# arjunchandra/paac

Measured on AMD Instinct MI355X. Metric: global env-steps/sec at 32 envs, t_max=5, Nature net; 1/2/4/8 MI355X, higher is better.
Workload: dtype f32; 1 GPU; breakout action set (A=4), NATURE net, 32 envs per GPU x 1 GPU, t_max=5, synthetic 84x84x4 u8 frames generated on device, sampler=numpy, hipGraph replay; envs_per_gpu=32, t_max=5, global_envs=32, parallelism=env-sharded dp1, no collective (one process)

## Files before the change

### __graft_entry__.py

```python
import os
import sys

ROOT = os.path.dirname(os.path.abspath(__file__))
if ROOT not in sys.path:
    sys.path.insert(0, ROOT)


USER_ARCHS = [
    "16,32,32,256",
    "32:8:4,64:5:2,64:3:1,512",
    "32:8:4,48:4:2,512",
    "16:8:4,16:4:1,256",
    "32:12:4,64:2:3,64:3:1,768",
    "16:4:2,32:1:1,48:5:5,1024",
    "32:8:4,64:4:2,64:8:1,512",
    "64:16:4,128:3:2,96:3:2,256",
]


def build():
    from concurrent.futures import ThreadPoolExecutor
    from paac_amd import build as b
    lib = b.build(verbose=False)
    with ThreadPoolExecutor(max_workers=4) as ex:
        list(ex.map(lambda spec: b.build_user_arch(*b.parse_user_arch(spec)), USER_ARCHS))
    from paac_amd import _lib
    _lib.load()
    assert os.path.exists(lib)
    import paac_amd.train


def smoke():
    import numpy as np
    import torch
    from oracle import network as onet
    from paac_amd import hip_ops
    assert torch.cuda.is_available(), "smoke() needs cuda:0"
    arch, A, B = "NATURE", 4, 40
    for weight_scale in (1.0, 3.5):
        rs = np.random.RandomState(0)
        params = {k: (v * weight_scale).astype(np.float32) for k, v in onet.init_params(arch, A, rs, dtype=np.float32).items()}
        states = rs.randint(0, 256, (B, 84, 84, 4)).astype(np.uint8)
        idx = rs.randint(0, A, B).astype(np.int32)
        y = rs.randn(B).astype(np.float32)
        adv = rs.randn(B).astype(np.float32)
        ctx = hip_ops.Context(1, A, max_batch=B)
        flat = np.zeros(ctx.layout["total"], dtype=np.float32)
        for t in ctx.layout["tensors"]:
            flat[t["offset"]:t["offset"] + t["size"]] = params[t["name"]].reshape(-1)
        p = torch.from_numpy(flat).cuda()
        s = torch.from_numpy(states).cuda()
        logits = torch.zeros((B, A), device="cuda")
        values = torch.zeros(B, device="cuda")
        grad = torch.zeros(ctx.layout["total"], device="cuda")
        ctx.forward(p, s, logits=logits, values=values)
        ctx.loss_backward(p, s, torch.from_numpy(idx).cuda(), torch.from_numpy(y).cuda(), torch.from_numpy(adv).cuda(), 0.02, grad)
        torch.cuda.synchronize()
        masks = {"a%d" % i: ctx.debug_activation(i, B).cpu().numpy() > 0 for i in (1, 2, 3)}
        masks["h"] = ctx.debug_activation(4, B).cpu().numpy() > 0
        L, g = onet.loss_and_grads(params, states, np.eye(A)[idx], y, adv, 0.02, arch, dtype=np.float64, relu_masks=masks)
        if weight_scale != 1.0:
            assert np.abs(L["logits"]).max() > 3.0 and np.abs(L["v"]).max() > 3.0
        assert np.abs(logits.cpu().numpy() - L["logits"]).max() < 1e-4
        assert np.abs(values.cpu().numpy() - L["v"]).max() < 1e-4
        gh = grad.cpu().numpy()
        gn = onet.global_norm(g)
        for t in ctx.layout["tensors"]:
            err = np.abs(gh[t["offset"]:t["offset"] + t["size"]] - g[t["name"]].reshape(-1)).max()
            assert err < 1e-4 * max(np.abs(g[t["name"]]).max(), 1e-3 * gn), (t["name"], err)
        ctx.close()
    print("smoke ok: logits/values within 1e-4, gradients within 1e-4 relative (initialisation-scale and trained-scale weights)")


if __name__ == "__main__":
    build()
    if len(sys.argv) > 1 and sys.argv[1] == "smoke":
        smoke()
```

### paac_amd/build.py

```python
import fcntl
import os
import subprocess
import sys
from concurrent.futures import ThreadPoolExecutor

HERE = os.path.dirname(os.path.abspath(__file__))
CSRC = os.path.join(HERE, "csrc")
LIB = os.path.join(HERE, "libpaac_hip.so")
SOURCES = ["api.hip", "net_fwd.hip", "net_bwd.hip", "misc.hip"]
HEADERS = sorted(f for f in os.listdir(CSRC) if f.endswith(".h")) + [os.path.join("..", "..", "include", "paac_hip.h")]
FLAGS = ["-O3", "-std=c++17", "--offload-arch=gfx950", "-fPIC", "-Wall", "-Wno-unused-function",
         "-Wno-unused-variable", "-Wno-unused-but-set-variable"]


def _stale(target, deps):
    if not os.path.exists(target):
        return True
    t = os.path.getmtime(target)
    return any(os.path.getmtime(d) > t for d in deps)


def build(force=False, verbose=True, extra_flags=(), lib_path=None, obj_suffix=""):
    lib = lib_path or LIB
    with open(lib + ".lock", "w") as lock:
        fcntl.flock(lock, fcntl.LOCK_EX)
        try:
            return _build_locked(force, verbose, extra_flags, lib, obj_suffix)
        finally:
            fcntl.flock(lock, fcntl.LOCK_UN)


def _build_locked(force, verbose, extra_flags, lib, obj_suffix):
    hipcc = os.environ.get("HIPCC", "/opt/rocm/bin/hipcc")
    hdrs = [os.path.join(CSRC, h) for h in HEADERS] + [os.path.abspath(__file__)]
    objs, jobs = [], []
    for src in SOURCES:
        s = os.path.join(CSRC, src)
        o = os.path.join(CSRC, src.replace(".hip", obj_suffix + ".o"))
        objs.append(o)
        if force or _stale(o, [s] + hdrs):
            jobs.append([hipcc] + FLAGS + list(extra_flags) + ["-c", s, "-o", o])

    def run(cmd):
        at = cmd.index("-o") + 1
        target = cmd[at]
        tmp = "%s.tmp.%d" % (target, os.getpid())
        cmd = cmd[:at] + [tmp] + cmd[at + 1:]
        try:
            _run(cmd)
            os.replace(tmp, target)
        finally:
            if os.path.exists(tmp):
                os.remove(tmp)

    def _run(cmd):
        if verbose:
            print(" ".join(cmd), flush=True)
        r = subprocess.run(cmd, capture_output=True, text=True)
        if r.returncode != 0:
            raise RuntimeError("hipcc failed:\n%s\n%s" % (" ".join(cmd), r.stderr[-8000:]))
        if verbose and r.stderr.strip():
            print(r.stderr[-4000:], file=sys.stderr)

    with ThreadPoolExecutor(max_workers=4) as ex:
        list(ex.map(run, jobs))
    if jobs or force or _stale(lib, objs):
        run([hipcc, "--offload-arch=gfx950", "-shared", "-fPIC", "-o", lib] + objs)
    return lib


def parse_user_arch(spec):
    parts = str(spec).split(",")
    convs = []
    for i, p in enumerate(parts[:-1]):
        v = [int(x) for x in p.split(":")]
        if len(v) == 1:
            if i >= len(FAMILY):
                raise ValueError("more than three layers in %r" % (spec,))
            v = [v[0]] + list(FAMILY[i])
        if len(v) != 3:
            raise ValueError("layer %r: expected filters or filters:size:stride" % (p,))
        convs.append(tuple(v))
    return convs, int(parts[-1])


FAMILY = [(8, 4), (4, 2), (3, 1)]


def user_arch_library(convs, fc):
    convs = [tuple(int(v) for v in c) for c in convs]
    tag = "_".join(str(f) for f, _, _ in convs) + "_%d" % fc
    if any((k, s) != FAMILY[i] for i, (_, k, s) in enumerate(convs)):
        tag += "_k" + "_".join("%dx%d" % (k, s) for _, k, s in convs)
    return os.path.join(HERE, "libpaac_hip_user_%s.so" % tag), "_user_" + tag


def build_user_arch(convs, fc, verbose=False):
    convs = [tuple(int(v) for v in c) for c in convs]
    if len(convs) not in (2, 3) or any(len(c) != 3 for c in convs):
        raise NotImplementedError("user architectures have two or three conv layers (filters, size, stride); got %r" % (convs,))
    if any(f % 16 or f < 16 for f, _, _ in convs) or fc % 256 or fc < 256:
        raise NotImplementedError("filter counts must be multiples of 16 and the fc width a multiple of 256 (MFMA tiles); "
                                  "got %r, fc %d" % (convs, fc))
    if any(k < 1 or s < 1 for _, k, s in convs):
        raise ValueError("kernel sizes and strides must be positive; got %r" % (convs,))
    if (convs[0][1] * 4) % 16:
        raise NotImplementedError("the first layer's kernel size must be 4, 8, 12 or 16 (kernel width x 4 input channels is "
                                  "read in MFMA K groups of 16); got %d" % convs[0][1])
    size = 84
    for _, k, s in convs:
        if size < k:
            raise ValueError("layer shapes %r leave no output (VALID convolutions over 84 x 84)" % (convs,))
        size = (size - k) // s + 1
    lib, suffix = user_arch_library(convs, fc)
    flags = ["-DPAAC_USER_ARCH", "-DPAAC_USER_NCONV=%d" % len(convs), "-DPAAC_USER_C1=%d" % convs[0][0],
             "-DPAAC_USER_C2=%d" % convs[1][0], "-DPAAC_USER_C3=%d" % (convs[2][0] if len(convs) == 3 else 0),
             "-DPAAC_USER_H=%d" % fc]
    layers = convs + [(0, 3, 1)] * (3 - len(convs))
    flags += ["-DPAAC_USER_K%d=%d" % (i + 1, k) for i, (_, k, _) in enumerate(layers)]
    flags += ["-DPAAC_USER_S%d=%d" % (i + 1, st) for i, (_, _, st) in enumerate(layers)]
    try:
        return build(verbose=verbose, extra_flags=flags, lib_path=lib, obj_suffix=suffix)
    except RuntimeError as exc:
        raise RuntimeError("building the user architecture %s (fc %d) failed: %s" % (convs, fc, exc)) from exc


if __name__ == "__main__":
    if "--user-arch" in sys.argv:
        spec = sys.argv[sys.argv.index("--user-arch") + 1]
        print(build_user_arch(*parse_user_arch(spec), verbose=True))
    elif "--stamps" in sys.argv or "--ksplit" in sys.argv:
        tag = ("_stamps" if "--stamps" in sys.argv else "") + ("_ksplit" if "--ksplit" in sys.argv else "")
        flags = (["-DPAAC_DMM_STAMPS"] if "--stamps" in sys.argv else []) + (["-DPAAC_T_ROLES=0"] if "--ksplit" in sys.argv else [])
        print(build(extra_flags=flags, lib_path=os.path.join(HERE, "libpaac_hip%s.so" % tag), obj_suffix=tag))
    else:
        print(build(force="--force" in sys.argv))
```

### paac_amd/csrc/net_fwd.hip

```cpp
#include "net_common.h"
#include "tower.h"
#include "tower2.h"
#include "fc_heads.h"
#include "gemm3.h"

namespace paac {

#ifdef PAAC_DMM_STAMPS
unsigned long long* g_tower_stamps = nullptr;
extern "C" void paac_debug_set_tower_stamps(unsigned long long* p) { g_tower_stamps = p; }
unsigned long long* g_stamps = nullptr;
int g_stamp_which = -1, g_stamp_calls = 0;
extern "C" void paac_debug_set_stamps(unsigned long long* p, int which) {
  g_stamps = p;
  g_stamp_which = which;
  g_stamp_calls = 0;
}
#endif

template <class G, bool U8, int NDIM, int EPI>
static int launch_fwd(const GemmArgs& g, Tune t, hipStream_t s) {
  constexpr int VN = (NDIM % 64 == 0) ? 4 : (NDIM % 32 == 0) ? 2 : 1;
  int cfg = t.cfg, ksplit = 1, xcd = t.xcd;
  if constexpr (EPI == EPI_SLAB) {
    ksplit = t.ksplit > 0 ? t.ksplit : 0;
    if (ksplit <= 0) {
      const long tiles = (long)((g.M + 15) / 16) * ((g.N + 16 * VN - 1) / (16 * VN));
      ksplit = pick_ksplit(tiles, 4, (g.K + 15) / 16, FC_SPLITS_MAX, 768);
    }
    if (ksplit > FC_SPLITS_MAX) ksplit = FC_SPLITS_MAX;
  }
  if (cfg < 0) {
    const long w = (long)((g.M + 15) / 16) * ((g.N + 16 * VN - 1) / (16 * VN)) * ksplit;
    cfg = (w <= 256) ? 0 : (w <= 1024) ? 3 : (w <= 4096) ? 4 : 5;
    if (U8) cfg += kExactBf16;
    xcd = -1;
  }
  if constexpr (U8) {
    if (cfg >= kExactBf16) {
      switch (cfg - kExactBf16) {
#define X(id, TM, NWM, WK, PF) \
  case id: launch_dmm<Dmm<G, U8, FRAG_K, FRAG_MN, TM, VN, NWM, 1, WK, 1, EPI, false, PF, 1>>(g, ksplit, ksplit, xcd, s); break;
        PAAC_FWD_CFGS(X)
#undef X
        default: break;
      }
      return ksplit;
    }
  }
  if constexpr (!U8 && VN == 4 && EPI == EPI_BIAS_RELU) {
    if (cfg >= kNarrow) {
      switch (cfg - kNarrow) {
#define X(id, TM, NWM, WK, PF) \
  case id: launch_dmm<Dmm<G, U8, FRAG_K, FRAG_MN, TM, 2, NWM, 1, WK, 1, EPI, false, PF>>(g, ksplit, ksplit, xcd, s); return ksplit;
        PAAC_FWD_NARROW_CFGS(X)
#undef X
        default: cfg -= kNarrow; break;
      }
    }
  }
  if (cfg >= kNarrow) cfg -= kNarrow;
  if constexpr (!U8) {
    if (cfg >= kSplitBf16) {
      switch (cfg - kSplitBf16) {
#define X(id, TM, NWM, WK, PF) \
  case id: launch_dmm<Dmm<G, U8, FRAG_K, FRAG_MN, TM, VN, NWM, 1, WK, 1, EPI, false, split_pf(PF), 2>>(g, ksplit, ksplit, xcd, s); return ksplit;
        PAAC_FWD_SPLIT_CFGS(X)
#undef X
        default: cfg -= kSplitBf16; break;
      }
    }
  }
  switch (cfg) {
#define X(id, TM, NWM, WK, PF) \
  case id: launch_dmm<Dmm<G, U8, FRAG_K, FRAG_MN, TM, VN, NWM, 1, WK, 1, EPI, false, PF>>(g, ksplit, ksplit, xcd, s); break;
    PAAC_FWD_CFGS(X)
#undef X
    default: break;
  }
  return ksplit;
}

static int launch_fc_gemm3(const float* x, const float* wf, float* slab, int batch, int K, int H, hipStream_t s) {
  static const int min_rows = env_int("PAAC_GEMM3_MIN_ROWS", 513);
  if (batch < min_rows || (K % 32) != 0) return 0;
  Gemm3Args a;
  memset(&a, 0, sizeof(a));
  a.A = x; a.lda = K;
  a.B = wf; a.ldb = H;
  a.out = slab; a.ldo = H;
  a.M = batch; a.N = H; a.K = K;
  using D = Gemm3<true, false, EPI_SLAB>;
  a.MB = (batch + D::TM - 1) / D::TM;
  a.NB = (H + D::TN - 1) / D::TN;
  const int stages = K / 32, tiles = a.MB * a.NB;
  int S = (256 + tiles / 2) / tiles;
  S = S < 1 ? 1 : (S > FC_SPLITS_MAX ? FC_SPLITS_MAX : S);
  a.stages_per_split = (stages + S - 1) / S;
  a.S = (stages + a.stages_per_split - 1) / a.stages_per_split;
  a.slab_stride = (long)batch * H;
  prof_mix(6);
  launch_k(gemm3_kernel<D>, dim3((unsigned)(a.MB * a.NB * a.S)), dim3(D::THREADS), s, PROF_WHOLE, a);
  return a.S;
}

size_t tower_pack_bytes() { return (size_t)kTowerPackAllVecs * sizeof(bf16x8); }
constexpr bool kTower2 = OtherNet::NCONV == 2 && OtherNet::C1 == 16 && OtherNet::C2 == 32 && OtherNet::FLAT == kT2Flat;
bool tower2_available() { return kTower2; }

int launch_pack_weights(paac_ctx* ctx, const float* params, hipStream_t s) {
  const paac_layout& L = ctx->layout;
  {
    const float* wf = params + L.offset[2 * ctx->spec.nconv];
    f32x4* out = reinterpret_cast<f32x4*>(ctx->fc_pack);
    if (ctx->cfg.arch == PAAC_ARCH_NATURE)
      launch_k(pack_fc_kernel<NatureNet::FLAT, NatureNet::H>, dim3((NatureNet::FLAT / 16) * (NatureNet::H / 16) * 64 / 256),
               dim3(256), s, PROF_NONE, wf, out);
    else
      launch_k(pack_fc_kernel<OtherNet::FLAT, OtherNet::H>, dim3((OtherNet::FLAT / 16) * (OtherNet::H / 16) * 64 / 256), dim3(256),
               s, PROF_NONE, wf, out);
  }
  if (ctx->tower2_on) {
    constexpr int threads2 = (8 * 1 + 8 * 2) * 64;
    launch_k(pack_tower2_kernel, dim3((threads2 + 255) / 256), dim3(256), s, PROF_NONE, params + L.offset[0], params + L.offset[2],
             reinterpret_cast<bf16x8*>(ctx->tower_pack));
    return 0;
  }
  if (!ctx->tower_on) return 0;
  constexpr int threads = (8 * 2 + 16 * 4 + 18 * 4) * 64;
  launch_k(pack_tower_kernel, dim3((threads + 255) / 256), dim3(256), s, PROF_NONE, params + L.offset[0], params + L.offset[2],
           params + L.offset[4], reinterpret_cast<bf16x8*>(ctx->tower_pack));
  return launch_pack_dgrad(ctx, params, s);
}

template <class G, bool KEEP>
static void launch_tower_variant(const TowerArgs& a, hipStream_t s) {
  launch_k(tower_kernel<G, KEEP>, dim3((unsigned)(a.batch * G::NR)), dim3(512), s, PROF_WHOLE, a);
}

static void launch_tower(paac_ctx* ctx, Workspace& W, const float* params, const uint8_t* states, int batch, bool keep,
                         bool packed3, hipStream_t s, Workspace* keepW = nullptr, int keep_row = 0) {
  const paac_layout& L = ctx->layout;
  TowerArgs a;
  a.states = states;
  const bf16x8* pk = reinterpret_cast<const bf16x8*>(ctx->tower_pack);
  a.w1p = pk;
  a.w2p = pk + kTowerW1Vecs;
  a.w3p = pk + kTowerW1Vecs + kTowerW2Vecs;
  a.b1 = params + L.offset[1];
  a.b2 = params + L.offset[3];
  a.b3 = params + L.offset[5];
  a.act1 = W.act[0];
  a.act2 = W.act[1];
  a.act3 = W.act[2];
  a.batch = batch;
  a.act3_packed = packed3 ? 1 : 0;
  a.act3_rows = nullptr;
  if (keepW) {
    keep = true;
    a.act1 = keepW->act[0] + (size_t)keep_row * 400 * NatureNet::C1;
    a.act2 = keepW->act[1] + (size_t)keep_row * 81 * NatureNet::C2;
    if (packed3) a.act3_rows = keepW->act[2] + (size_t)keep_row * NatureNet::FLAT;
    else a.act3 = keepW->act[2] + (size_t)keep_row * NatureNet::FLAT;
  }
#ifdef PAAC_DMM_STAMPS
  a.stamps = g_tower_stamps;
#endif
  const int force = ctx->tune[OP_CONV_TOWER][batch_class(batch)].cfg;
  int regions = (8 * batch <= 256) ? 8 : (4 * batch <= 256) ? 4 : (2 * batch <= 256) ? 2 : 1;
  if (force == 1 || force == 2 || force == 4 || force == 8) regions = force;
  if (regions == 8) {
    if (keep) launch_tower_variant<TowerGeom<4, 2>, true>(a, s);
    else launch_tower_variant<TowerGeom<4, 2>, false>(a, s);
  } else if (regions == 4) {
    if (keep) launch_tower_variant<TowerGeom<4, 4>, true>(a, s);
    else launch_tower_variant<TowerGeom<4, 4>, false>(a, s);
  } else if (regions == 2) {
    if (keep) launch_tower_variant<TowerGeom<4, 7>, true>(a, s);
    else launch_tower_variant<TowerGeom<4, 7>, false>(a, s);
  } else {
    if (keep) launch_tower_variant<TowerGeom<7, 7>, true>(a, s);
    else launch_tower_variant<TowerGeom<7, 7>, false>(a, s);
  }
}

template <class G, bool KEEP>
static void launch_tower2_variant(const Tower2Args& a, hipStream_t s) {
  launch_k(tower2_kernel<G, KEEP>, dim3((unsigned)(a.batch * G::NR)), dim3(512), s, PROF_WHOLE, a);
}

static void launch_tower2(paac_ctx* ctx, Workspace& W, const float* params, const uint8_t* states, int batch, bool keep,
                          bool packed2, hipStream_t s, Workspace* keepW = nullptr, int keep_row = 0) {
  const paac_layout& L = ctx->layout;
  Tower2Args a;
  a.states = states;
  const bf16x8* pk = reinterpret_cast<const bf16x8*>(ctx->tower_pack);
  a.w1p = pk;
  a.w2p = pk + kT2W1Vecs;
  a.b1 = params + L.offset[1];
  a.b2 = params + L.offset[3];
  a.act1 = W.act[0];
  a.act2 = W.act[1];
  a.batch = batch;
  a.act2_packed = packed2 ? 1 : 0;
  a.act2_rows = nullptr;
  if (keepW) {
    keep = true;
    a.act1 = keepW->act[0] + (size_t)keep_row * 400 * 16;
    if (packed2) a.act2_rows = keepW->act[1] + (size_t)keep_row * kT2Flat;
    else a.act2 = keepW->act[1] + (size_t)keep_row * kT2Flat;
  }
  const int force = ctx->tune[OP_CONV_TOWER][batch_class(batch)].cfg;
  int regions = (9 * batch <= 256) ? 9 : (4 * batch <= 256) ? 4 : 1;
  if (force == 1 || force == 4 || force == 9) regions = force;
  if (regions == 9) {
    if (keep) launch_tower2_variant<Tower2Geom<3, 3>, true>(a, s);
    else launch_tower2_variant<Tower2Geom<3, 3>, false>(a, s);
  } else if (regions == 4) {
    if (keep) launch_tower2_variant<Tower2Geom<5, 5>, true>(a, s);
    else launch_tower2_variant<Tower2Geom<5, 5>, false>(a, s);
  } else {
    if (keep) launch_tower2_variant<Tower2Geom<9, 9>, true>(a, s);
    else launch_tower2_variant<Tower2Geom<9, 9>, false>(a, s);
  }
}

template <class NT>
static int forward_impl(paac_ctx* ctx, int wsi, const float* params, const uint8_t* states, int batch, float* logits,
                        float* probs, float* values, const PhiloxArgs& ph, const SynthStepArgs& st, hipStream_t s,
                        bool defer_heads = false, bool trunk_only = false) {
  const paac_layout& L = ctx->layout;
  Workspace& W = ctx->ws[wsi];
  ctx->last_ws = wsi;
  const int cls = batch_class(batch);
  const int A = ctx->cfg.num_actions;
  int t = 0;
  const float* w1 = params + L.offset[t++];
  const float* b1 = params + L.offset[t++];
  const float* w2 = params + L.offset[t++];
  const float* b2 = params + L.offset[t++];
  const float* w3 = nullptr;
  const float* b3 = nullptr;
  if constexpr (NT::NCONV == 3) {
    w3 = params + L.offset[t++];
    b3 = params + L.offset[t++];
  }
  const float* wf = params + L.offset[t++];
  const float* bf = params + L.offset[t++];
  const float* wa = params + L.offset[t++];
// ... 316 lines not shown
```

### paac_amd/csrc/tower.h

```cpp
#pragma once
#include "dmm.h"

namespace paac {

struct TowerArgs {
  const uint8_t* states;
  const bf16x8* w1p;
  const bf16x8* w2p;
  const bf16x8* w3p;
  const float* b1;
  const float* b2;
  const float* b3;
  float* act1;
  float* act2;
  float* act3;
  int act3_packed;
  float* act3_rows;
  int batch;
#ifdef PAAC_DMM_STAMPS
  unsigned long long* stamps;
#endif
};

#ifdef PAAC_DMM_STAMPS
#define TOWER_STAMP(i)                                                                                      \
  do {                                                                                                      \
    __builtin_amdgcn_sched_barrier(0);                                                                      \
    if (p.stamps && lane == 0)                                                                              \
      p.stamps[((long)blockIdx.x * 8 + wave) * 12 + (i)] =                                                  \
          ((i) == 0 || (i) == 11) ? (unsigned long long)wall_clock64() : (unsigned long long)clock64();    \
    __builtin_amdgcn_sched_barrier(0);                                                                      \
  } while (0)
#else
#define TOWER_STAMP(i)
#endif

#ifndef PAAC_T_KS2
#define PAAC_T_KS2 2
#endif
#ifndef PAAC_T_KS3
#define PAAC_T_KS3 2
#endif
#ifndef PAAC_T_ROLES
#define PAAC_T_ROLES 1
#endif
constexpr int kTowerW1Vecs = 8 * 2 * 3 * 64, kTowerW2Vecs = 16 * 4 * 3 * 64, kTowerW3Vecs = 18 * 4 * 3 * 64;
constexpr int kTowerPackVecs = kTowerW1Vecs + kTowerW2Vecs + kTowerW3Vecs;
constexpr int kDgradW3Vecs = 18 * 4 * 3 * 64, kDgradW2Vecs = 4 * 8 * 2 * 3 * 64;
constexpr int kTowerPackAllVecs = kTowerPackVecs + kDgradW3Vecs + kDgradW2Vecs;

__device__ __forceinline__ void split3_store(const float (&x)[8], bf16x8* dst ) {
  bf16x8 h, m, l;
  split3_bf16(x, h, m, l);
  dst[0] = h;
  dst[64] = m;
  dst[128] = l;
}

static __global__ __launch_bounds__(256) void pack_tower_kernel(const float* __restrict__ w1, const float* __restrict__ w2,
                                                         const float* __restrict__ w3, bf16x8* __restrict__ out) {
  int i = blockIdx.x * 256 + threadIdx.x;
  const float* w;
  int cout, ctiles;
  bf16x8* dst;
  if (i < 8 * 2 * 64) {
    w = w1; cout = 32; ctiles = 2; dst = out;
  } else if (i < 8 * 2 * 64 + 16 * 4 * 64) {
    i -= 8 * 2 * 64;
    w = w2; cout = 64; ctiles = 4; dst = out + kTowerW1Vecs;
  } else if (i < 8 * 2 * 64 + 16 * 4 * 64 + 18 * 4 * 64) {
    i -= 8 * 2 * 64 + 16 * 4 * 64;
    w = w3; cout = 64; ctiles = 4; dst = out + kTowerW1Vecs + kTowerW2Vecs;
  } else {
    return;
  }
  const int lane = i & 63, unit = i >> 6;
  const int ct = unit % ctiles, s = unit / ctiles;
  const int ch = lane & 15, kq = lane >> 4;
  float x[8];
#pragma unroll
  for (int j = 0; j < 8; ++j) x[j] = w[(long)(32 * s + 8 * kq + j) * cout + 16 * ct + ch];
  split3_store(x, dst + (long)unit * 192 + lane);
}

template <int R3H_, int R3W_>
struct TowerGeom {
  static constexpr int R3H = R3H_, R3W = R3W_;
  static constexpr int R2H = R3H + 2, R2W = R3W + 2;
  static constexpr int R1H = 2 * R2H + 2, R1W = 2 * R2W + 2;
  static constexpr int RIH = 4 * R1H + 4, RIW = 4 * R1W + 4;
  static constexpr int NRY = (7 + R3H - 1) / R3H, NRX = (7 + R3W - 1) / R3W, NR = NRY * NRX;
  static constexpr int P1 = R1H * R1W, P2 = R2H * R2W, P3 = R3H * R3W;
  static constexpr int PT1 = (P1 + 15) / 16, PT2 = (P2 + 15) / 16, PT3 = (P3 + 15) / 16;
  static constexpr int S1 = 80, S2 = 160;
  static constexpr int PL1 = P1 * S1, PL2 = P2 * S2;
  static constexpr bool ROLES = PAAC_T_ROLES != 0 && PT2 <= PAAC_T_KS2 && PT3 <= PAAC_T_KS3;
  static constexpr bool KSPLIT2 = !ROLES && ((PT2 % 2) != 0 || PT2 <= PAAC_T_KS2);
  static constexpr bool KSPLIT3 = !ROLES && ((PT3 % 2) != 0 || PT3 <= PAAC_T_KS3);
  static constexpr int NT1 = (PT1 + 3) / 4;
  static constexpr int NT2 = (KSPLIT2 || ROLES) ? PT2 : PT2 / 2, NT3 = (KSPLIT3 || ROLES) ? PT3 : PT3 / 2;
  static constexpr int PF1 = 8, PF2 = (KSPLIT2 || ROLES) ? 8 : 6, PF3 = ROLES ? 8 : KSPLIT3 ? 9 : 6;
  static constexpr int IN_BYTES = RIH * RIW * 8;
  static constexpr int SCR2 = KSPLIT2 ? 4 * NT2 * 1024 : 0;
  static constexpr int FRONT = (IN_BYTES > 3 * PL2 + SCR2) ? IN_BYTES : 3 * PL2 + SCR2;
  static constexpr int FRONT_AL = (FRONT + 15) / 16 * 16;
  static constexpr int W1_BYTES = kTowerW1Vecs * 16;
  static constexpr bool W1_LDS = FRONT_AL + 3 * PL1 + W1_BYTES <= 160 * 1024;
  static constexpr int LDS_BYTES = FRONT_AL + 3 * PL1 + (W1_LDS ? W1_BYTES : 0);
  static_assert(RIW % 4 == 0, "input rows are staged 4 pixels (16 bytes) at a time");
  static_assert(!KSPLIT3 || 4 * NT3 * 1024 <= 3 * PL1, "conv3 K-split partials reuse the conv1 planes");
  static_assert(LDS_BYTES <= 160 * 1024, "LDS budget");
};

__device__ __forceinline__ f32x4 mfma_bf16(const bf16x8 a, const bf16x8 b, const f32x4 c) {
  return __builtin_amdgcn_mfma_f32_16x16x32_bf16(a, b, c, 0, 0, 0);
}

struct NoHook {
  __device__ __forceinline__ void operator()(int) const {}
};

template <int NS, int NT, int CT, int BP, int BPL, int PF_, class KOFF, bool DB = true, int KSETS = 0>
struct WaveGemm {
  static constexpr int PF = PF_ < NS ? PF_ : NS;
  static constexpr int RING = PF < NS ? PF + 1 : NS;
  bf16x8 a[RING][3];
  const bf16x8* wl;
  int ct, sg_mul, sg_add;

  __device__ __forceinline__ void set(const bf16x8* wl_, const int ct_, const int sg_mul_, const int sg_add_) {
    wl = wl_; ct = ct_; sg_mul = sg_mul_; sg_add = sg_add_;
  }
  __device__ __forceinline__ void load_a(const int slot, const int i) {
    const bf16x8* src = wl + (long)((sg_mul * i + sg_add) * CT + ct) * 192;
#pragma unroll
    for (int pl = 0; pl < 3; ++pl) a[slot][pl] = src[pl * 64];
  }
  __device__ __forceinline__ void prologue_step(const int j) {
    if (j >= 0 && j < PF) load_a(j, j);
  }
  __device__ __forceinline__ void prologue(const bf16x8* wl_, const int ct_, const int sg_mul_, const int sg_add_) {
    set(wl_, ct_, sg_mul_, sg_add_);
#pragma unroll
    for (int i = 0; i < PF; ++i) load_a(i, i);
    __builtin_amdgcn_sched_barrier(0);
  }
  __device__ __forceinline__ void read_b(bf16x8 (&b)[NT][BP], const char* lds_b, const unsigned (&bb)[NT], const int i) {
    const int ko = KOFF::at(i);
#pragma unroll
    for (int t = 0; t < NT; ++t)
#pragma unroll
      for (int pl = 0; pl < BP; ++pl) b[t][pl] = *reinterpret_cast<const bf16x8*>(lds_b + bb[t] + ko + pl * BPL);
  }
  template <class Hook = NoHook>
  __device__ __forceinline__ void run(const char* __restrict__ lds_b, const unsigned (&bb)[NT], f32x4 (&acc)[NT],
                                      Hook hook = Hook()) {
    bf16x8 b[DB ? 2 : 1][NT][BP];
    f32x4 acc2[KSETS > 0 ? NT : 1];
    if constexpr (KSETS > 0) {
#pragma unroll
      for (int t = 0; t < NT; ++t) acc2[t] = (f32x4){0.f, 0.f, 0.f, 0.f};
    }
    if constexpr (DB) read_b(b[0], lds_b, bb, 0);
#pragma unroll
    for (int i = 0; i < NS; ++i) {
      if (i + PF < NS) load_a((i + PF) % RING, i + PF);
      hook(i);
      if constexpr (DB) {
        if (i + 1 < NS) read_b(b[(i + 1) & 1], lds_b, bb, i + 1);
      } else {
        read_b(b[0], lds_b, bb, i);
      }
      __builtin_amdgcn_sched_barrier(0);
      const int slot = i % RING;
      constexpr int NB = DB ? 2 : 1;
      if constexpr (BP == 1) {
#pragma unroll
        for (int pl = 2; pl >= 0; --pl)
#pragma unroll
          for (int t = 0; t < NT; ++t) acc[t] = mfma_bf16(a[slot][pl], b[i % NB][t][0], acc[t]);
      } else if constexpr (KSETS > 0) {
        const bf16x8(&bs)[NT][BP] = b[i % NB];
        f32x4(&as)[NT] = ((i / KSETS) & 1) ? acc2 : acc;
#pragma unroll
        for (int t = 0; t < NT; ++t) as[t] = mfma_bf16(a[slot][2], bs[t][0], as[t]);
#pragma unroll
        for (int t = 0; t < NT; ++t) as[t] = mfma_bf16(a[slot][1], bs[t][1], as[t]);
#pragma unroll
        for (int t = 0; t < NT; ++t) as[t] = mfma_bf16(a[slot][0], bs[t][2], as[t]);
#pragma unroll
        for (int t = 0; t < NT; ++t) as[t] = mfma_bf16(a[slot][1], bs[t][0], as[t]);
#pragma unroll
        for (int t = 0; t < NT; ++t) as[t] = mfma_bf16(a[slot][0], bs[t][1], as[t]);
#pragma unroll
        for (int t = 0; t < NT; ++t) as[t] = mfma_bf16(a[slot][0], bs[t][0], as[t]);
      } else {
#pragma unroll
        for (int t = 0; t < NT; ++t) {
          const bf16x8(&bt)[BP] = b[i % NB][t];
          acc[t] = mfma_bf16(a[slot][2], bt[0], acc[t]);
          acc[t] = mfma_bf16(a[slot][1], bt[1], acc[t]);
          acc[t] = mfma_bf16(a[slot][0], bt[2], acc[t]);
          acc[t] = mfma_bf16(a[slot][1], bt[0], acc[t]);
          acc[t] = mfma_bf16(a[slot][0], bt[1], acc[t]);
          acc[t] = mfma_bf16(a[slot][0], bt[0], acc[t]);
        }
      }
      __builtin_amdgcn_sched_barrier(0);
    }
    if constexpr (KSETS > 0) {
#pragma unroll
      for (int t = 0; t < NT; ++t) acc[t] += acc2[t];
    }
  }
};

template <int PLANE_STRIDE>
__device__ __forceinline__ void store_split4(char* dst, const f32x4 v) {
  unsigned xb[4], r1b[4], r2b[4];
#pragma unroll
  for (int e = 0; e < 4; ++e) {
    const float x = v[e];
    xb[e] = __builtin_bit_cast(unsigned, x);
    const float r1 = x - __builtin_bit_cast(float, xb[e] & 0xFFFF0000u);
    r1b[e] = __builtin_bit_cast(unsigned, r1);
    const float r2 = r1 - __builtin_bit_cast(float, r1b[e] & 0xFFFF0000u);
    r2b[e] = __builtin_bit_cast(unsigned, r2);
  }
  *reinterpret_cast<u32x2*>(dst) = (u32x2){pack_hi16(xb[0], xb[1]), pack_hi16(xb[2], xb[3])};
  *reinterpret_cast<u32x2*>(dst + PLANE_STRIDE) = (u32x2){pack_hi16(r1b[0], r1b[1]), pack_hi16(r1b[2], r1b[3])};
  *reinterpret_cast<u32x2*>(dst + 2 * PLANE_STRIDE) = (u32x2){pack_hi16(r2b[0], r2b[1]), pack_hi16(r2b[2], r2b[3])};
}

template <int P, int RW, int S, int PL, int C>
__device__ __forceinline__ void store_kept_rows(const char* __restrict__ planes, float* __restrict__ img ,
                                                const int img_w, const int htid) {
  constexpr int V = C / 4, N = P * V;
#pragma unroll
  for (int i0 = 0; i0 < N; i0 += 256) {
    const int i = i0 + htid;
    if (i0 + 256 > N && i >= N) break;
    const int pi = i / V, c4 = i - pi * V;
    const char* src = planes + pi * S + c4 * 8;
    const u32x2 h = *reinterpret_cast<const u32x2*>(src), m = *reinterpret_cast<const u32x2*>(src + PL),
                l = *reinterpret_cast<const u32x2*>(src + 2 * PL);
    f32x4 v;
#pragma unroll
    for (int q = 0; q < 2; ++q) {
      v[2 * q] = (__builtin_bit_cast(float, l[q] << 16) + __builtin_bit_cast(float, m[q] << 16)) + __builtin_bit_cast(float, h[q] << 16);
      v[2 * q + 1] = (__builtin_bit_cast(float, l[q] & 0xFFFF0000u) + __builtin_bit_cast(float, m[q] & 0xFFFF0000u)) +
                     __builtin_bit_cast(float, h[q] & 0xFFFF0000u);
    }
    const int y = pi / RW, x = pi - y * RW;
    *reinterpret_cast<f32x4*>(img + ((size_t)y * img_w + x) * C + 4 * c4) = v;
  }
}

template <class G>
struct Koff1 {
  __device__ static constexpr int at(int i) { return i * G::RIW * 8; }
};
template <class G>
struct Koff2 {
  __device__ static constexpr int at(int i) { return ((i / 4) * G::R1W + (i % 4)) * G::S1; }
};
template <class G>
struct Koff3Half {
  __device__ static constexpr int at(int i) { return ((i / 3) * G::R2W + (i % 3)) * G::S2; }
};
template <class G>
struct Koff3Full {
  __device__ static constexpr int at(int i) { return (((i / 2) / 3) * G::R2W + ((i / 2) % 3)) * G::S2 + (i % 2) * 64; }
};

template <class G, bool WRITE_ALL>
__global__ __launch_bounds__(512) void tower_kernel(const TowerArgs p) {
  __shared__ __attribute__((aligned(16))) char lds[G::LDS_BYTES];
  char* const lds_in = lds;
  char* const lds_a2 = lds;
  char* const lds_s2 = lds + 3 * G::PL2;
  char* const lds_a1 = lds + G::FRONT_AL;
  char* const lds_s3 = lds_a1;
  char* const lds_w1 = lds_a1 + 3 * G::PL1;

  const int tid = threadIdx.x;
  const int lane = tid & 63;
  const int wave = __builtin_amdgcn_readfirstlane(tid >> 6);
  const int li = lane & 15, kq = lane >> 4;
  const int b = blockIdx.x / G::NR, reg = blockIdx.x % G::NR;
  const int ry = reg / G::NRX, rx = reg % G::NRX;
  const int y3n = ry * G::R3H, x3n = rx * G::R3W;
  const int y3a = y3n < 7 - G::R3H ? y3n : 7 - G::R3H, x3a = x3n < 7 - G::R3W ? x3n : 7 - G::R3W;
  const int y1a = 2 * y3a, x1a = 2 * x3a;

  TOWER_STAMP(0);
  TOWER_STAMP(1);
  WaveGemm<8, G::NT1, 2, 1, 0, G::W1_LDS ? 2 : G::PF1, Koff1<G>> g1;
  WaveGemm<G::KSPLIT2 ? 8 : 16, G::NT2, 4, 3, G::PL1, G::PF2, Koff2<G>, true, G::ROLES ? 8 : 0> g2;
  const bool gemm_wave = !G::ROLES || wave < 4;

  {
    constexpr int VROW = G::RIW / 4, NV = G::RIH * VROW, ITERS = (NV + 511) / 512;
    const uint8_t* src = p.states + (size_t)b * 28224 + ((8 * y3a) * 84 + 8 * x3a) * 4;
    uint4 v[ITERS];
#pragma unroll
    for (int it = 0; it < ITERS; ++it) {
      const int i = tid + it * 512;
      const int r = i / VROW, c4 = i - r * VROW;
      if (i < NV) v[it] = *reinterpret_cast<const uint4*>(src + (r * 84 + 4 * c4) * 4);
    }
    constexpr int W1V = G::W1_LDS ? kTowerW1Vecs / 512 : 1;
    bf16x8 w1v[W1V];
    if constexpr (G::W1_LDS) {
#pragma unroll
      for (int it = 0; it < W1V; ++it) w1v[it] = p.w1p[tid + it * 512];
    } else {
      g1.prologue(p.w1p + lane, wave & 1, 1, 0);
    }
#pragma unroll
    for (int it = 0; it < ITERS; ++it) {
      const int i = tid + it * 512;
      if (i < NV) {
        const unsigned w[4] = {v[it].x, v[it].y, v[it].z, v[it].w};
        u32x4 o[2];
#pragma unroll
        for (int px = 0; px < 4; ++px) {
          unsigned f[4];
#pragma unroll
          for (int c = 0; c < 4; ++c) f[c] = __builtin_bit_cast(unsigned, (float)((w[px] >> (8 * c)) & 255u));
          o[px >> 1][2 * (px & 1)] = pack_hi16(f[0], f[1]);
          o[px >> 1][2 * (px & 1) + 1] = pack_hi16(f[2], f[3]);
        }
        u32x4* dst = reinterpret_cast<u32x4*>(lds_in + (size_t)i * 32);
        dst[0] = o[0];
        dst[1] = o[1];
      }
    }
    if constexpr (G::W1_LDS) {
#pragma unroll
      for (int it = 0; it < W1V; ++it) reinterpret_cast<bf16x8*>(lds_w1)[tid + it * 512] = w1v[it];
    }
  }
  TOWER_STAMP(2);
  __syncthreads();
  TOWER_STAMP(3);

  {
    const int ct = wave & 1, grp = wave >> 1;
    unsigned bb[G::NT1];
    int pix[G::NT1];
#pragma unroll
    for (int j = 0; j < G::NT1; ++j) {
      const int tile = grp + 4 * j;
      const int pi = 16 * tile + li;
      const bool ok = (tile < G::PT1) && (pi < G::P1);
      pix[j] = ok ? pi : -1;
      const int pc = ok ? pi : 0;
      const int y1 = pc / G::R1W, x1 = pc - y1 * G::R1W;
      bb[j] = (unsigned)(((4 * y1) * G::RIW + 4 * x1 + 2 * kq) * 8);
    }
    f32x4 acc[G::NT1];
#pragma unroll
    for (int j = 0; j < G::NT1; ++j) acc[j] = (f32x4){0.f, 0.f, 0.f, 0.f};
    const f32x4 bias = *reinterpret_cast<const f32x4*>(p.b1 + 16 * ct + 4 * kq);
    if constexpr (G::W1_LDS) {
      g2.set(p.w2p + lane, wave & 3, 1, G::KSPLIT2 ? 8 * (wave >> 2) : 0);
      g1.prologue(reinterpret_cast<const bf16x8*>(lds_w1) + lane, ct, 1, 0);
      g1.run(lds_in, bb, acc, [&](const int i) { if (gemm_wave) g2.prologue_step(i); });
#pragma unroll
      for (int j = 8; j < decltype(g2)::PF; ++j)
        if (gemm_wave) g2.prologue_step(j);
      __builtin_amdgcn_sched_barrier(0);
    } else {
      g1.run(lds_in, bb, acc);
    }
    TOWER_STAMP(4);
    if constexpr (!G::W1_LDS) {
      if (gemm_wave) g2.prologue(p.w2p + lane, wave & 3, 1, G::KSPLIT2 ? 8 * (wave >> 2) : 0);
    }
#pragma unroll
    for (int j = 0; j < G::NT1; ++j) {
      if (pix[j] < 0) continue;
      f32x4 v;
#pragma unroll
      for (int e = 0; e < 4; ++e) v[e] = fmaxf(acc[j][e] * kInputScale + bias[e], 0.f);
      if constexpr (WRITE_ALL && !G::ROLES) {
        const int y1 = pix[j] / G::R1W, x1 = pix[j] - y1 * G::R1W;
        *reinterpret_cast<f32x4*>(p.act1 + ((size_t)(b * 20 + y1a + y1) * 20 + x1a + x1) * 32 + 16 * ct + 4 * kq) = v;
      }
      store_split4<G::PL1>(lds_a1 + pix[j] * G::S1 + (16 * ct + 4 * kq) * 2, v);
    }
  }
  TOWER_STAMP(5);
  __syncthreads();
  TOWER_STAMP(6);

  WaveGemm<9, G::NT3, 4, 3, G::PL2, G::PF3, Koff3Half<G>> g3h;
  WaveGemm<18, G::NT3, 4, 3, G::PL2, G::PF3, Koff3Full<G>, true, G::ROLES ? 1 : 0> g3f;
  if (gemm_wave) {
    const int ct = wave & 3, half = wave >> 2;
    unsigned bb[G::NT2];
    int pix[G::NT2];
#pragma unroll
    for (int j = 0; j < G::NT2; ++j) {
      const int tile = G::KSPLIT2 ? j : half * G::NT2 + j;
      const int pi = 16 * tile + li;
      const bool ok = pi < G::P2;
      pix[j] = ok ? pi : -1;
      const int pc = ok ? pi : 0;
      const int y2 = pc / G::R2W, x2 = pc - y2 * G::R2W;
      bb[j] = (unsigned)(((2 * y2) * G::R1W + 2 * x2) * G::S1 + kq * 16 +
                         (G::KSPLIT2 ? half * (2 * G::R1W * G::S1) : 0));
    }
    f32x4 acc[G::NT2];
#pragma unroll
    for (int j = 0; j < G::NT2; ++j) acc[j] = (f32x4){0.f, 0.f, 0.f, 0.f};
    const f32x4 bias = *reinterpret_cast<const f32x4*>(p.b2 + 16 * ct + 4 * kq);
    constexpr int NS2 = G::KSPLIT2 ? 8 : 16;
    if constexpr (G::KSPLIT3) {
      constexpr int LEAD = decltype(g3h)::PF - NS2;
      g3h.set(p.w3p + lane, ct, 2, half);
#pragma unroll
      for (int j = 0; j < LEAD; ++j) g3h.prologue_step(j);
      g2.run(lds_a1, bb, acc, [&](const int i) { g3h.prologue_step(i + LEAD); });
    } else {
      constexpr int LEAD = decltype(g3f)::PF - NS2;
      g3f.set(p.w3p + lane, ct, 1, 0);
#pragma unroll
      for (int j = 0; j < LEAD; ++j) g3f.prologue_step(j);
      g2.run(lds_a1, bb, acc, [&](const int i) { g3f.prologue_step(i + LEAD); });
    }
    TOWER_STAMP(7);
    constexpr int OWN0 = G::KSPLIT2 ? (G::NT2 + 1) / 2 : G::NT2;
    const int j_lo = (G::KSPLIT2 && half == 1) ? OWN0 : 0, j_hi = (G::KSPLIT2 && half == 0) ? OWN0 : G::NT2;
    if constexpr (G::KSPLIT2) {
      f32x4* scr = reinterpret_cast<f32x4*>(lds_s2);
#pragma unroll
      for (int j = 0; j < G::NT2; ++j)
        if (j < j_lo || j >= j_hi) scr[(ct * G::NT2 + j) * 64 + lane] = acc[j];
      __syncthreads();
#pragma unroll
      for (int j = 0; j < G::NT2; ++j)
        if (j >= j_lo && j < j_hi) acc[j] += scr[(ct * G::NT2 + j) * 64 + lane];
    }
#pragma unroll
    for (int j = 0; j < G::NT2; ++j) {
      if (j < j_lo || j >= j_hi || pix[j] < 0) continue;
      f32x4 v;
#pragma unroll
      for (int e = 0; e < 4; ++e) v[e] = fmaxf(acc[j][e] + bias[e], 0.f);
      if constexpr (WRITE_ALL && !G::ROLES) {
        const int y2 = pix[j] / G::R2W, x2 = pix[j] - y2 * G::R2W;
        *reinterpret_cast<f32x4*>(p.act2 + ((size_t)(b * 9 + y3a + y2) * 9 + x3a + x2) * 64 + 16 * ct + 4 * kq) = v;
      }
      store_split4<G::PL2>(lds_a2 + pix[j] * G::S2 + (16 * ct + 4 * kq) * 2, v);
    }
  } else {
    if constexpr (WRITE_ALL)
      store_kept_rows<G::P1, G::R1W, G::S1, G::PL1, 32>(lds_a1, p.act1 + ((size_t)(b * 20 + y1a) * 20 + x1a) * 32, 20, tid - 256);
    TOWER_STAMP(7);
  }
  __syncthreads();
  TOWER_STAMP(8);

  if (gemm_wave) {
    const int ct = wave & 3, half = wave >> 2;
    unsigned bb[G::NT3];
    int pix[G::NT3];
#pragma unroll
    for (int j = 0; j < G::NT3; ++j) {
      const int tile = G::KSPLIT3 ? j : half * G::NT3 + j;
      const int pi = 16 * tile + li;
      const bool ok = pi < G::P3;
      pix[j] = ok ? pi : -1;
      const int pc = ok ? pi : 0;
      const int y3 = pc / G::R3W, x3 = pc - y3 * G::R3W;
      bb[j] = (unsigned)((y3 * G::R2W + x3) * G::S2 + kq * 16 + (G::KSPLIT3 ? half * 64 : 0));
    }
    f32x4 acc[G::NT3];
#pragma unroll
    for (int j = 0; j < G::NT3; ++j) acc[j] = (f32x4){0.f, 0.f, 0.f, 0.f};
    const f32x4 bias = *reinterpret_cast<const f32x4*>(p.b3 + 16 * ct + 4 * kq);
    if constexpr (G::KSPLIT3) g3h.run(lds_a2, bb, acc);
    else g3f.run(lds_a2, bb, acc);
    TOWER_STAMP(9);
    if constexpr (G::KSPLIT3) {
      f32x4* scr = reinterpret_cast<f32x4*>(lds_s3);
      if (half == 1) {
#pragma unroll
        for (int j = 0; j < G::NT3; ++j) scr[(ct * G::NT3 + j) * 64 + lane] = acc[j];
      }
      __syncthreads();
      if (half == 0) {
#pragma unroll
        for (int j = 0; j < G::NT3; ++j) acc[j] += scr[(ct * G::NT3 + j) * 64 + lane];
      }
    }
    if (!G::KSPLIT3 || half == 0) {
      const int dup_y = y3n - y3a, dup_x = x3n - x3a;
#pragma unroll
      for (int j = 0; j < G::NT3; ++j) {
        if (pix[j] < 0) continue;
        const int y3 = pix[j] / G::R3W, x3 = pix[j] - y3 * G::R3W;
        if (y3 < dup_y || x3 < dup_x) continue;
        f32x4 v;
#pragma unroll
        for (int e = 0; e < 4; ++e) v[e] = fmaxf(acc[j][e] + bias[e], 0.f);
        const int k0 = ((y3a + y3) * 7 + x3a + x3) * 64 + 16 * ct + 4 * kq;
        if (p.act3_packed)
          *reinterpret_cast<f32x4*>(p.act3 + ((((size_t)(b >> 4) * (3136 / 16) + (k0 >> 4)) * 64 + ((k0 >> 2) & 3) * 16 + (b & 15)) << 2)) = v;
        else
          *reinterpret_cast<f32x4*>(p.act3 + (size_t)b * 3136 + k0) = v;
        if (p.act3_rows) *reinterpret_cast<f32x4*>(p.act3_rows + (size_t)b * 3136 + k0) = v;
      }
    }
  } else {
    if constexpr (WRITE_ALL)
      store_kept_rows<G::P2, G::R2W, G::S2, G::PL2, 64>(lds_a2, p.act2 + ((size_t)(b * 9 + y3a) * 9 + x3a) * 64, 9, tid - 256);
    TOWER_STAMP(9);
  }
  TOWER_STAMP(10);
  TOWER_STAMP(11);
}

}
```

Before: 742,200 env-steps/s.

## Interleave LDS and weight loads across MFMAs and pad conv1 LDS rows

Adds a 'spread' path to the wave GEMM for the lone-wave roles configuration. It reads B fragments two k-steps ahead and uses sched_group_barrier to put one LDS read or global weight load behind each MFMA, so memory latency is hidden under matrix math instead of arriving in bursts. It also pads each conv1 activation row in LDS by 32 bytes to shift bank mapping, likely to reduce bank conflicts, and updates the offsets, index and store helpers to match. A blocked variant library without spreading is built alongside for comparison, and kstamp timing probes are added under a debug flag.

```diff
diff --git a/__graft_entry__.py b/__graft_entry__.py
--- a/__graft_entry__.py
+++ b/__graft_entry__.py
@@ -22,6 +22,7 @@
     from concurrent.futures import ThreadPoolExecutor
     from paac_amd import build as b
     lib = b.build(verbose=False)
+    b.build_blocked()
     with ThreadPoolExecutor(max_workers=4) as ex:
         list(ex.map(lambda spec: b.build_user_arch(*b.parse_user_arch(spec)), USER_ARCHS))
     from paac_amd import _lib
diff --git a/paac_amd/build.py b/paac_amd/build.py
--- a/paac_amd/build.py
+++ b/paac_amd/build.py
@@ -11,6 +11,17 @@
 HEADERS = sorted(f for f in os.listdir(CSRC) if f.endswith(".h")) + [os.path.join("..", "..", "include", "paac_hip.h")]
 FLAGS = ["-O3", "-std=c++17", "--offload-arch=gfx950", "-fPIC", "-Wall", "-Wno-unused-function",
          "-Wno-unused-variable", "-Wno-unused-but-set-variable"]
+
+
+VARIANTS = {"--stamps": "-DPAAC_DMM_STAMPS", "--ksplit": "-DPAAC_T_ROLES=0", "--blocked": "-DPAAC_T_SPREAD=0"}
+BLOCKED_LIB = os.path.join(HERE, "libpaac_hip_blocked.so")
+
+
+def build_blocked(verbose=False):
+    srcs = [os.path.join(CSRC, f) for f in SOURCES + HEADERS] + [os.path.abspath(__file__)]
+    if os.path.exists(BLOCKED_LIB) and not _stale(BLOCKED_LIB, srcs):
+        return BLOCKED_LIB
+    return build(verbose=verbose, extra_flags=[VARIANTS["--blocked"]], lib_path=BLOCKED_LIB, obj_suffix="_blocked")
 
 
 def _stale(target, deps):
@@ -129,9 +140,10 @@
     if "--user-arch" in sys.argv:
         spec = sys.argv[sys.argv.index("--user-arch") + 1]
         print(build_user_arch(*parse_user_arch(spec), verbose=True))
-    elif "--stamps" in sys.argv or "--ksplit" in sys.argv:
-        tag = ("_stamps" if "--stamps" in sys.argv else "") + ("_ksplit" if "--ksplit" in sys.argv else "")
-        flags = (["-DPAAC_DMM_STAMPS"] if "--stamps" in sys.argv else []) + (["-DPAAC_T_ROLES=0"] if "--ksplit" in sys.argv else [])
+    elif any(f in sys.argv for f in VARIANTS):
+        on = [f for f in VARIANTS if f in sys.argv]
+        tag = "".join("_" + f[2:] for f in on)
+        flags = [VARIANTS[f] for f in on]
         print(build(extra_flags=flags, lib_path=os.path.join(HERE, "libpaac_hip%s.so" % tag), obj_suffix=tag))
     else:
         print(build(force="--force" in sys.argv))
diff --git a/paac_amd/csrc/net_fwd.hip b/paac_amd/csrc/net_fwd.hip
--- a/paac_amd/csrc/net_fwd.hip
+++ b/paac_amd/csrc/net_fwd.hip
@@ -9,6 +9,8 @@
 #ifdef PAAC_DMM_STAMPS
 unsigned long long* g_tower_stamps = nullptr;
 extern "C" void paac_debug_set_tower_stamps(unsigned long long* p) { g_tower_stamps = p; }
+unsigned long long* g_tower_kstamps = nullptr;
+extern "C" void paac_debug_set_tower_kstamps(unsigned long long* p) { g_tower_kstamps = p; }
 unsigned long long* g_stamps = nullptr;
 int g_stamp_which = -1, g_stamp_calls = 0;
 extern "C" void paac_debug_set_stamps(unsigned long long* p, int which) {
@@ -165,6 +167,7 @@
   }
 #ifdef PAAC_DMM_STAMPS
   a.stamps = g_tower_stamps;
+  a.kstamps = g_tower_kstamps;
 #endif
   const int force = ctx->tune[OP_CONV_TOWER][batch_class(batch)].cfg;
   int regions = (8 * batch <= 256) ? 8 : (4 * batch <= 256) ? 4 : (2 * batch <= 256) ? 2 : 1;
diff --git a/paac_amd/csrc/tower.h b/paac_amd/csrc/tower.h
--- a/paac_amd/csrc/tower.h
+++ b/paac_amd/csrc/tower.h
@@ -19,6 +19,7 @@
   int batch;
 #ifdef PAAC_DMM_STAMPS
   unsigned long long* stamps;
+  unsigned long long* kstamps;
 #endif
 };
 
@@ -43,6 +44,12 @@
 #endif
 #ifndef PAAC_T_ROLES
 #define PAAC_T_ROLES 1
+#endif
+#ifndef PAAC_T_SPREAD
+#define PAAC_T_SPREAD 1
+#endif
+#ifndef PAAC_T_RPAD
+#define PAAC_T_RPAD PAAC_T_SPREAD
 #endif
 constexpr int kTowerW1Vecs = 8 * 2 * 3 * 64, kTowerW2Vecs = 16 * 4 * 3 * 64, kTowerW3Vecs = 18 * 4 * 3 * 64;
 constexpr int kTowerPackVecs = kTowerW1Vecs + kTowerW2Vecs + kTowerW3Vecs;
@@ -93,8 +100,13 @@
   static constexpr int P1 = R1H * R1W, P2 = R2H * R2W, P3 = R3H * R3W;
   static constexpr int PT1 = (P1 + 15) / 16, PT2 = (P2 + 15) / 16, PT3 = (P3 + 15) / 16;
   static constexpr int S1 = 80, S2 = 160;
-  static constexpr int PL1 = P1 * S1, PL2 = P2 * S2;
+  static constexpr int PL2 = P2 * S2;
   static constexpr bool ROLES = PAAC_T_ROLES != 0 && PT2 <= PAAC_T_KS2 && PT3 <= PAAC_T_KS3;
+  static constexpr bool SPREAD = ROLES && PAAC_T_SPREAD != 0;
+  static constexpr int RP1 = (ROLES && PAAC_T_RPAD != 0) ? 32 : 0;
+  static constexpr int ROW1 = R1W * S1 + RP1;
+  static constexpr int PL1 = R1H * ROW1;
+  static_assert(RP1 == 0 || (R1W == 10 && R2W == 4 && P2 % 16 == 8), "RP1 was worked out for the 4x2 regions");
   static constexpr bool KSPLIT2 = !ROLES && ((PT2 % 2) != 0 || PT2 <= PAAC_T_KS2);
   static constexpr bool KSPLIT3 = !ROLES && ((PT3 % 2) != 0 || PT3 <= PAAC_T_KS3);
   static constexpr int NT1 = (PT1 + 3) / 4;
@@ -118,13 +130,32 @@
 
 struct NoHook {
   __device__ __forceinline__ void operator()(int) const {}
-};
-
-template <int NS, int NT, int CT, int BP, int BPL, int PF_, class KOFF, bool DB = true, int KSETS = 0>
+  __device__ static constexpr int loads(int) { return 0; }
+};
+
+#ifdef PAAC_DMM_STAMPS
+#define TOWER_KSTAMP(step, slot)                                                                            \
+  do {                                                                                                      \
+    if (i == (step) && kst) {                                                                               \
+      __builtin_amdgcn_sched_barrier(0);                                                                    \
+      if ((threadIdx.x & 63) == 0) kst[(slot)] = (unsigned long long)clock64();                             \
+      __builtin_amdgcn_sched_barrier(0);                                                                    \
+    }                                                                                                       \
+  } while (0)
+#else
+#define TOWER_KSTAMP(step, slot)
+#endif
+
+template <int NS, int NT, int CT, int BP, int BPL, int PF_, class KOFF, bool DB = true, int KSETS = 0, bool SPREAD = false>
 struct WaveGemm {
   static constexpr int PF = PF_ < NS ? PF_ : NS;
   static constexpr int RING = PF < NS ? PF + 1 : NS;
+  static_assert(!SPREAD || (KSETS > 0 && BP == 3 && DB && PF < NS), "SPREAD: the lone-wave path only");
+  static_assert(!SPREAD || NT * BP + 3 <= 6 * NT, "SPREAD: one request behind each MFMA of a k-step");
   bf16x8 a[RING][3];
+#ifdef PAAC_DMM_STAMPS
+  unsigned long long* kst = nullptr;
+#endif
   const bf16x8* wl;
   int ct, sg_mul, sg_add;
 
@@ -139,6 +170,7 @@
   __device__ __forceinline__ void prologue_step(const int j) {
     if (j >= 0 && j < PF) load_a(j, j);
   }
+  __device__ static constexpr int prologue_loads(const int j) { return (j >= 0 && j < PF) ? 3 : 0; }
   __device__ __forceinline__ void prologue(const bf16x8* wl_, const int ct_, const int sg_mul_, const int sg_add_) {
     set(wl_, ct_, sg_mul_, sg_add_);
 #pragma unroll
@@ -155,6 +187,10 @@
   template <class Hook = NoHook>
   __device__ __forceinline__ void run(const char* __restrict__ lds_b, const unsigned (&bb)[NT], f32x4 (&acc)[NT],
                                       Hook hook = Hook()) {
+    if constexpr (SPREAD) {
+      run_spread(lds_b, bb, acc, hook);
+      return;
+    }
     bf16x8 b[DB ? 2 : 1][NT][BP];
     f32x4 acc2[KSETS > 0 ? NT : 1];
     if constexpr (KSETS > 0) {
@@ -164,6 +200,7 @@
     if constexpr (DB) read_b(b[0], lds_b, bb, 0);
 #pragma unroll
     for (int i = 0; i < NS; ++i) {
+      TOWER_KSTAMP(NS / 2, 0);
       if (i + PF < NS) load_a((i + PF) % RING, i + PF);
       hook(i);
       if constexpr (DB) {
@@ -172,6 +209,7 @@
         read_b(b[0], lds_b, bb, i);
       }
       __builtin_amdgcn_sched_barrier(0);
+      TOWER_KSTAMP(NS / 2, 1);
       const int slot = i % RING;
       constexpr int NB = DB ? 2 : 1;
       if constexpr (BP == 1) {
@@ -207,12 +245,68 @@
         }
       }
       __builtin_amdgcn_sched_barrier(0);
+      TOWER_KSTAMP(NS / 2, 2);
     }
     if constexpr (KSETS > 0) {
 #pragma unroll
       for (int t = 0; t < NT; ++t) acc[t] += acc2[t];
     }
   }
+
+  template <class Hook>
+  __device__ __forceinline__ void run_spread(const char* __restrict__ lds_b, const unsigned (&bb)[NT], f32x4 (&acc)[NT],
+                                             Hook hook) {
+    constexpr int LEAD = 2, NB = LEAD + 1, NM = 6 * NT;
+    bf16x8 b[NB][NT][BP];
+    f32x4 acc2[NT];
+#pragma unroll
+    for (int t = 0; t < NT; ++t) acc2[t] = (f32x4){0.f, 0.f, 0.f, 0.f};
+#pragma unroll
+    for (int j = 0; j < LEAD && j < NS; ++j) read_b(b[j], lds_b, bb, j);
+    __builtin_amdgcn_sched_barrier(0);
+#pragma unroll
+    for (int i = 0; i < NS; ++i) {
+      TOWER_KSTAMP(NS / 2, 0);
+      TOWER_KSTAMP(NS / 2, 1);
+      const int nds = (i + LEAD < NS) ? NT * BP : 0;
+      const int nvm = ((i + PF < NS) ? 3 : 0) + Hook::loads(i);
+      if (i + LEAD < NS) read_b(b[(i + LEAD) % NB], lds_b, bb, i + LEAD);
+      if (i + PF < NS) load_a((i + PF) % RING, i + PF);
+      hook(i);
+      const int slot = i % RING;
+      const bf16x8(&bs)[NT][BP] = b[i % NB];
+      f32x4(&as)[NT] = ((i / KSETS) & 1) ? acc2 : acc;
+#pragma unroll
+      for (int t = 0; t < NT; ++t) as[t] = mfma_bf16(a[slot][2], bs[t][0], as[t]);
+#pragma unroll
+      for (int t = 0; t < NT; ++t) as[t] = mfma_bf16(a[slot][1], bs[t][1], as[t]);
+#pragma unroll
+      for (int t = 0; t < NT; ++t) as[t] = mfma_bf16(a[slot][0], bs[t][2], as[t]);
+#pragma unroll
+      for (int t = 0; t < NT; ++t) as[t] = mfma_bf16(a[slot][1], bs[t][0], as[t]);
+#pragma unroll
+      for (int t = 0; t < NT; ++t) as[t] = mfma_bf16(a[slot][0], bs[t][1], as[t]);
+#pragma unroll
+      for (int t = 0; t < NT; ++t) as[t] = mfma_bf16(a[slot][0], bs[t][0], as[t]);
+#pragma unroll
+      for (int k = 0; k < NM; ++k) {
+        __builtin_amdgcn_sched_group_barrier(0x008, 1, 0);
+        if (k < nds) __builtin_amdgcn_sched_group_barrier(0x100, 1, 0);
+        else if (k >= NM - nvm) __builtin_amdgcn_sched_group_barrier(0x020, 1, 0);
+      }
+      __builtin_amdgcn_sched_barrier(0);
+      TOWER_KSTAMP(NS / 2, 2);
+    }
+#pragma unroll
+    for (int t = 0; t < NT; ++t) acc[t] += acc2[t];
+  }
+};
+
+template <class GN, int LEAD>
+struct WindowHook {
+  GN& g;
+  __device__ __forceinline__ void operator()(const int i) const { g.prologue_step(i + LEAD); }
+  __device__ static constexpr int loads(const int i) { return GN::prologue_loads(i + LEAD); }
 };
 
 template <int PLANE_STRIDE>
@@ -232,7 +326,7 @@
   *reinterpret_cast<u32x2*>(dst + 2 * PLANE_STRIDE) = (u32x2){pack_hi16(r2b[0], r2b[1]), pack_hi16(r2b[2], r2b[3])};
 }
 
-template <int P, int RW, int S, int PL, int C>
+template <int P, int RW, int S, int PL, int C, int ROW = 0>
 __device__ __forceinline__ void store_kept_rows(const char* __restrict__ planes, float* __restrict__ img ,
                                                 const int img_w, const int htid) {
   constexpr int V = C / 4, N = P * V;
@@ -241,7 +335,8 @@
     const int i = i0 + htid;
     if (i0 + 256 > N && i >= N) break;
     const int pi = i / V, c4 = i - pi * V;
-    const char* src = planes + pi * S + c4 * 8;
+    const int y = pi / RW, x = pi - y * RW;
+    const char* src = planes + (ROW ? y * ROW + x * S : pi * S) + c4 * 8;
     const u32x2 h = *reinterpret_cast<const u32x2*>(src), m = *reinterpret_cast<const u32x2*>(src + PL),
                 l = *reinterpret_cast<const u32x2*>(src + 2 * PL);
     f32x4 v;
@@ -251,7 +346,6 @@
       v[2 * q + 1] = (__builtin_bit_cast(float, l[q] & 0xFFFF0000u) + __builtin_bit_cast(float, m[q] & 0xFFFF0000u)) +
                      __builtin_bit_cast(float, h[q] & 0xFFFF0000u);
     }
-    const int y = pi / RW, x = pi - y * RW;
     *reinterpret_cast<f32x4*>(img + ((size_t)y * img_w + x) * C + 4 * c4) = v;
   }
 }
@@ -262,7 +356,7 @@
 };
 template <class G>
 struct Koff2 {
-  __device__ static constexpr int at(int i) { return ((i / 4) * G::R1W + (i % 4)) * G::S1; }
+  __device__ static constexpr int at(int i) { return (i / 4) * G::ROW1 + (i % 4) * G::S1; }
 };
 template <class G>
 struct Koff3Half {
@@ -296,7 +390,7 @@
   TOWER_STAMP(0);
   TOWER_STAMP(1);
   WaveGemm<8, G::NT1, 2, 1, 0, G::W1_LDS ? 2 : G::PF1, Koff1<G>> g1;
-  WaveGemm<G::KSPLIT2 ? 8 : 16, G::NT2, 4, 3, G::PL1, G::PF2, Koff2<G>, true, G::ROLES ? 8 : 0> g2;
+  WaveGemm<G::KSPLIT2 ? 8 : 16, G::NT2, 4, 3, G::PL1, G::PF2, Koff2<G>, true, G::ROLES ? 8 : 0, G::SPREAD> g2;
   const bool gemm_wave = !G::ROLES || wave < 4;
 
   {
@@ -388,7 +482,9 @@
         const int y1 = pix[j] / G::R1W, x1 = pix[j] - y1 * G::R1W;
         *reinterpret_cast<f32x4*>(p.act1 + ((size_t)(b * 20 + y1a + y1) * 20 + x1a + x1) * 32 + 16 * ct + 4 * kq) = v;
       }
-      store_split4<G::PL1>(lds_a1 + pix[j] * G::S1 + (16 * ct + 4 * kq) * 2, v);
+      int at1 = pix[j] * G::S1;
+      if constexpr (G::RP1 != 0) at1 += (pix[j] / G::R1W) * G::RP1;
+      store_split4<G::PL1>(lds_a1 + at1 + (16 * ct + 4 * kq) * 2, v);
     }
   }
   TOWER_STAMP(5);
@@ -396,7 +492,13 @@
   TOWER_STAMP(6);
 
   WaveGemm<9, G::NT3, 4, 3, G::PL2, G::PF3, Koff3Half<G>> g3h;
-  WaveGemm<18, G::NT3, 4, 3, G::PL2, G::PF3, Koff3Full<G>, true, G::ROLES ? 1 : 0> g3f;
+  WaveGemm<18, G::NT3, 4, 3, G::PL2, G::PF3, Koff3Full<G>, true, G::ROLES ? 1 : 0, G::SPREAD> g3f;
+#ifdef PAAC_DMM_STAMPS
+  if (G::ROLES && gemm_wave && p.kstamps) {
+    g2.kst = p.kstamps + ((long)blockIdx.x * 4 + wave) * 8;
+    g3f.kst = g2.kst + 3;
+  }
+#endif
   if (gemm_wave) {
     const int ct = wave & 3, half = wave >> 2;
     unsigned bb[G::NT2];
@@ -407,9 +509,9 @@
       const int pi = 16 * tile + li;
       const bool ok = pi < G::P2;
       pix[j] = ok ? pi : -1;
-      const int pc = ok ? pi : 0;
+      const int pc = ok ? pi : G::RP1 != 0 ? pi - 8 : 0;
       const int y2 = pc / G::R2W, x2 = pc - y2 * G::R2W;
-      bb[j] = (unsigned)(((2 * y2) * G::R1W + 2 * x2) * G::S1 + kq * 16 +
+      bb[j] = (unsigned)(((2 * y2) * G::R1W + 2 * x2) * G::S1 + (2 * y2) * G::RP1 + kq * 16 +
                          (G::KSPLIT2 ? half * (2 * G::R1W * G::S1) : 0));
     }
     f32x4 acc[G::NT2];
@@ -428,7 +530,8 @@
       g3f.set(p.w3p + lane, ct, 1, 0);
 #pragma unroll
       for (int j = 0; j < LEAD; ++j) g3f.prologue_step(j);
-      g2.run(lds_a1, bb, acc, [&](const int i) { g3f.prologue_step(i + LEAD); });
+      if constexpr (G::SPREAD) g2.run(lds_a1, bb, acc, WindowHook<decltype(g3f), LEAD>{g3f});
+      else g2.run(lds_a1, bb, acc, [&](const int i) { g3f.prologue_step(i + LEAD); });
     }
     TOWER_STAMP(7);
     constexpr int OWN0 = G::KSPLIT2 ? (G::NT2 + 1) / 2 : G::NT2;
@@ -457,7 +560,7 @@
     }
   } else {
     if constexpr (WRITE_ALL)
-      store_kept_rows<G::P1, G::R1W, G::S1, G::PL1, 32>(lds_a1, p.act1 + ((size_t)(b * 20 + y1a) * 20 + x1a) * 32, 20, tid - 256);
+      store_kept_rows<G::P1, G::R1W, G::S1, G::PL1, 32, G::RP1 != 0 ? G::ROW1 : 0>(lds_a1, p.act1 + ((size_t)(b * 20 + y1a) * 20 + x1a) * 32, 20, tid - 256);
     TOWER_STAMP(7);
   }
   __syncthreads();
```

After: 741,500 env-steps/s. About the same (-0.1%).
